# ziyangwang007/CV-SSL-MIS

Hardware: AMD Instinct MI355X
Metric: training images-or-volumes/sec/node (Mean-Teacher step) (higher is better)
Workload: dtype f32

## Files before the change

cv-ssl-mis_amd/csrc/norm_act.hip:

```cpp
#include "common.h"
#include <type_traits>

namespace {

struct Geo {
    int N, C, per_sample;
    long long S;
    long long x_bs;
    int P;
    int nchunks;
    int G;
    int cg;
};

__host__ __device__ inline int pick_P(long long S) {
    long long p = (S + 16383) / 16384;
    if (p < 1) p = 1;
    if (p > 32) p = 32;
    return (int)p;
}

Geo make_geo(int N, int C, long long S, long long x_bs, int per_sample, int cg = 1) {
    Geo g;
    g.N = N; g.C = C; g.S = S; g.x_bs = x_bs; g.per_sample = per_sample; g.cg = cg;
// ... 3 lines not shown
    return g;
}

struct ResArgs {
    const float* r; long long r_bs;
    float* dr; long long dr_bs; int dr_acc;
    int post;
};

struct DropCfg {
    float p;
    unsigned salt;
    const MisStepState* st;
    const float* mask;
};

__device__ __forceinline__ void drop_scale4(const DropCfg& d, unsigned long long idx, unsigned chan, float s[4]) {
    if (d.mask) {
        const float4 m = *reinterpret_cast<const float4*>(d.mask + idx);
        s[0] = m.x; s[1] = m.y; s[2] = m.z; s[3] = m.w;
        return;
    }
    const unsigned long long seed = d.st->seed, off = d.st->offset;
    const float keep = 1.f / (1.f - d.p);
    uint32_t r[4];
    if (d.salt >> 31) {
        mis_philox4((uint32_t)chan, 0x3D0D3D0Du, d.salt, (uint32_t)off, (uint32_t)seed,
                    (uint32_t)(seed >> 32) ^ (uint32_t)(off >> 32), r);
        const float v = mis_u01(r[0]) >= d.p ? keep : 0.f;
        s[0] = s[1] = s[2] = s[3] = v;
// ... 163 lines not shown
                                                        float* __restrict__ y, long long y_bs, ResArgs ra) {
    const int c = blockIdx.y, n = blockIdx.z;
    const int grp = g.per_sample ? (n * g.C + c) / g.cg : c;
    const float sc = (gamma ? gamma[c] : 1.f) * rstd[grp];
    const float sh = (beta ? beta[c] : 0.f) - mean[grp] * sc;
    const float* __restrict__ xb = x + (long long)n * g.x_bs + (long long)c * g.S;
    float* __restrict__ yb = y + (long long)n * y_bs + (long long)c * g.S;
    const unsigned long long lbase = ((unsigned long long)n * g.C + c) * g.S;
    const long long units = g.S >> 2;
    const bool drop = d.p > 0.f;
#pragma unroll
    for (int i = 0; i < APPLY_U; ++i) {
        const long long u = ((long long)blockIdx.x * APPLY_U + i) * 256 + threadIdx.x;
        if (u >= units) break;
        const float4 q = *reinterpret_cast<const float4*>(xb + u * 4);
        float v[4] = {q.x * sc + sh, q.y * sc + sh, q.z * sc + sh, q.w * sc + sh};
        float4 rq = make_float4(0.f, 0.f, 0.f, 0.f);
        if constexpr (RES) {
            rq = *reinterpret_cast<const float4*>(ra.r + (long long)n * ra.r_bs + (long long)c * g.S + u * 4);
            if (!ra.post) { v[0] += rq.x; v[1] += rq.y; v[2] += rq.z; v[3] += rq.w; }
        }
#pragma unroll
        for (int j = 0; j < 4; ++j) v[j] = v[j] > 0.f ? v[j] : v[j] * slope;
        if constexpr (RES) {
            if (ra.post) { v[0] += rq.x; v[1] += rq.y; v[2] += rq.z; v[3] += rq.w; }
        }
        if (drop) {
            float s[4];
            drop_scale4(d, lbase + u * 4, (unsigned)(n * g.C + c), s);
#pragma unroll
            for (int j = 0; j < 4; ++j) v[j] *= s[j];
        }
        *reinterpret_cast<float4*>(yb + u * 4) = make_float4(v[0], v[1], v[2], v[3]);
    }
}

template <int PZ>
__global__ __launch_bounds__(256) void apply_fwd_pool_kernel(const float* __restrict__ x, Geo g,
                                                             const float* __restrict__ mean,
                                                             const float* __restrict__ rstd,
                                                             const float* __restrict__ gamma,
                                                             const float* __restrict__ beta, float slope, DropCfg d,
                                                             float* __restrict__ y, long long y_bs,
                                                             float* __restrict__ pooled, long long p_bs,
                                                             unsigned char* __restrict__ idx, int H, int W) {
    const int Ho = H >> 1, Wo = W >> 1, Wq = Wo >> 2;
    const int pl = blockIdx.x * 256 + threadIdx.x;
    if (pl >= Ho * Wq) return;
    const int zo = blockIdx.y, nc = blockIdx.z;
    const int n = nc / g.C, c = nc - n * g.C;
    const int yo = pl / Wq, xq = pl - yo * Wq;
    const int grp = g.per_sample ? (n * g.C + c) / g.cg : c;
    const float sc = (gamma ? gamma[c] : 1.f) * rstd[grp];
    const float sh = (beta ? beta[c] : 0.f) - mean[grp] * sc;
    const float* __restrict__ xb = x + (long long)n * g.x_bs + (long long)c * g.S;
    float* __restrict__ yb = y + (long long)n * y_bs + (long long)c * g.S;
    const unsigned long long lbase = ((unsigned long long)n * g.C + c) * g.S;
    const bool drop = d.p > 0.f;
    float best[4] = {-INFINITY, -INFINITY, -INFINITY, -INFINITY};
    unsigned bi[4] = {0, 0, 0, 0};
#pragma unroll
    for (int dz = 0; dz < PZ; ++dz)
#pragma unroll
        for (int dy = 0; dy < 2; ++dy) {
            const unsigned e = (unsigned)(((zo * PZ + dz) * H + (yo * 2 + dy)) * W + xq * 8);
            float v[8];
#pragma unroll
            for (int h = 0; h < 2; ++h) {
                const float4 q = *reinterpret_cast<const float4*>(xb + e + 4 * h);
                float t[4] = {q.x * sc + sh, q.y * sc + sh, q.z * sc + sh, q.w * sc + sh};
#pragma unroll
                for (int j = 0; j < 4; ++j) t[j] = t[j] > 0.f ? t[j] : t[j] * slope;
                if (drop) {
                    float s4[4];
                    drop_scale4(d, lbase + e + 4 * h, (unsigned)(n * g.C + c), s4);
#pragma unroll
                    for (int j = 0; j < 4; ++j) t[j] *= s4[j];
                }
                *reinterpret_cast<float4*>(yb + e + 4 * h) = make_float4(t[0], t[1], t[2], t[3]);
#pragma unroll
                for (int j = 0; j < 4; ++j) v[4 * h + j] = t[j];
            }
#pragma unroll
            for (int j = 0; j < 4; ++j)
#pragma unroll
                for (int dx = 0; dx < 2; ++dx) {
                    const float t = v[2 * j + dx];
                    if (t > best[j] || t != t) { best[j] = t; bi[j] = dz * 4 + dy * 2 + dx; }
                }
        }
    const long long So = (long long)gridDim.y * Ho * Wo;
    const unsigned o = (unsigned)((zo * Ho + yo) * Wo + xq * 4);
    *reinterpret_cast<float4*>(pooled + (long long)n * p_bs + (long long)c * So + o) =
        make_float4(best[0], best[1], best[2], best[3]);
    *reinterpret_cast<unsigned*>(idx + (long long)nc * So + o) = bi[0] | (bi[1] << 8) | (bi[2] << 16) | (bi[3] << 24);
}

template <bool DACC, bool RES = false>
__global__ __launch_bounds__(256) void bwd_partial_kernel(const float* __restrict__ x, Geo g,
                                                          const float* __restrict__ da, long long da_bs,
                                                          const float* __restrict__ mean,
                                                          const float* __restrict__ rstd,
                                                          const float* __restrict__ gamma,
                                                          const float* __restrict__ beta, float slope, DropCfg d,
                                                          float2* __restrict__ part, PoolGrad pg, ResArgs ra) {
    __shared__ double red[8];
    const int p = blockIdx.x, k = blockIdx.y, grp = blockIdx.z;
    const int n = g.per_sample ? grp / g.C : k;
    const int c = g.per_sample ? grp % g.C : grp;
    const int sg = g.per_sample ? grp / g.cg : grp;
// ... 414 lines not shown
                                hipStream_t stream) {
    return mis_norm_act_fwd_g(x, x_bs, y, y_bs, N, C, S, per_sample, 1, mean, rstd, gamma, beta, slope, drop_p,
                              drop_salt, state, drop_mask, stream);
}

extern "C" int mis_norm_act_fwd_pool(const float* x, long long x_bs, float* y, long long y_bs, float* pooled,
                                     long long p_bs, unsigned char* idx, int N, int C, int D, int H, int W,
                                     int per_sample, int cg, const float* mean, const float* rstd, const float* gamma,
                                     const float* beta, float slope, float drop_p, unsigned drop_salt,
                                     const MisStepState* state, const float* drop_mask, hipStream_t stream) {
    if (D <= 0 || H <= 0 || W <= 0) return MIS_ERR_ARG;
    const long long S = (long long)D * H * W;
    int st = check_geo(x, N, C, S, x_bs);
    if (st) return st;
    if (cg < 1 || C % cg != 0 || (cg > 1 && !per_sample)) return MIS_ERR_ARG;
    if (!y || !pooled || !idx || !mean || !rstd || y_bs < (long long)C * S) return MIS_ERR_ARG;
    if (W % 8 || H % 2 || (D > 1 && D % 2) || S >= (1LL << 31)) return MIS_ERR_UNSUPPORTED;
    const int pz = D > 1 ? 2 : 1, Do = D / pz;
    const long long So = (long long)Do * (H / 2) * (W / 2);
    if (p_bs < (long long)C * So) return MIS_ERR_ARG;
    if (y_bs % 4 || p_bs % 4 || !aligned16(y) || !aligned16(pooled) || ((uintptr_t)idx & 3)) return MIS_ERR_UNSUPPORTED;
    if (drop_p < 0.f || drop_p >= 1.f || (drop_p > 0.f && !state && !drop_mask)) return MIS_ERR_ARG;
    if (Do > 65535 || (long long)N * C > 65535) return MIS_ERR_UNSUPPORTED;
    const Geo g = make_geo(N, C, S, x_bs, per_sample, cg);
    const DropCfg d{drop_p, drop_salt, state, drop_mask};
    const dim3 grid((unsigned)(((H / 2) * (W / 8) + 255) / 256), Do, N * C);
    if (pz == 2)
        hipLaunchKernelGGL(apply_fwd_pool_kernel<2>, grid, dim3(256), 0, stream, x, g, mean, rstd, gamma, beta, slope, d, y,
                           y_bs, pooled, p_bs, idx, H, W);
    else
        hipLaunchKernelGGL(apply_fwd_pool_kernel<1>, grid, dim3(256), 0, stream, x, g, mean, rstd, gamma, beta, slope, d, y,
                           y_bs, pooled, p_bs, idx, H, W);
    return mis_launch_status();
}

namespace {
int norm_act_bwd_impl(const float* x, long long x_bs, const float* da, long long da_bs, float* dx, long long dx_bs,
                      int N, int C, long long S, int per_sample, int cg, int no_norm, const float* mean,
                      const float* rstd, const float* gamma, const float* beta, float slope, float drop_p,
                      unsigned drop_salt, const MisStepState* state, const float* drop_mask, float* dgamma,
                      float* dbeta, int accumulate_affine, void* workspace, long long workspace_bytes,
                      const PoolGrad& pg, hipStream_t stream, const ResArgs& ra = ResArgs{}) {
    if (S % 4 != 0) {
        if (ra.r) return MIS_ERR_UNSUPPORTED;
        int st = check_geo_small(x, N, C, S, x_bs);
        if (st) return st;
        if (!da || !dx || !mean || !rstd || da_bs < (long long)C * S || dx_bs < (long long)C * S) return MIS_ERR_ARG;
// ... 171 lines not shown

struct HeadArgs {
    const float* x; long long x_bs;
    int N, K, per_sample;
    long long S;
    const float* mean; const float* rstd; const float* gamma; const float* beta;
    float slope;
    const float* w; const float* b;
    float* logits; long long l_bs;
    const float* dl; long long dl_bs;
    float* dx; long long dx_bs;
    float2* part;
    const float2* sums;
    float* hpart;
    int P;
};

template <int C, bool MASK>
__device__ __forceinline__ unsigned long long head_drop_bits(const DropCfg& d, int n, long long S, long long u) {
    unsigned long long bits = ~0ull;
    if (!MASK && d.p > 0.f) {
        bits = 0;
#pragma unroll 1
        for (int c = 0; c < C; ++c) {
            float s[4];
            drop_scale4(d, ((unsigned long long)n * C + c) * S + u * 4, (unsigned)(n * C + c), s);
#pragma unroll
            for (int j = 0; j < 4; ++j) bits |= (unsigned long long)(s[j] != 0.f) << (4 * c + j);
        }
    }
// ... 24 lines not shown
template <int C, int K, bool MASK>
__global__ __launch_bounds__(256) void head_fwd_fused_kernel(const HeadArgs a, DropCfg d) {
    __shared__ float sc[C], sh[C], sw[K * C];
    const int n = blockIdx.y;
    head_coeffs<C>(a, n, sc, sh);
    for (int i = threadIdx.x; i < K * C; i += 256) sw[i] = a.w[i];
    __syncthreads();
    const long long units = a.S >> 2, u = (long long)blockIdx.x * 256 + threadIdx.x;
    if (u >= units) return;
    const float* __restrict__ xb = a.x + (long long)n * a.x_bs + u * 4;
    float4 q[C];
#pragma unroll
    for (int c = 0; c < C; ++c) q[c] = *reinterpret_cast<const float4*>(xb + (long long)c * a.S);
    const float keep = d.p > 0.f ? 1.f / (1.f - d.p) : 1.f;
    const unsigned long long bits = head_drop_bits<C, MASK>(d, n, a.S, u);
    float acc[K][4];
#pragma unroll
    for (int k = 0; k < K; ++k) {
        const float bk = a.b ? a.b[k] : 0.f;
#pragma unroll
        for (int j = 0; j < 4; ++j) acc[k][j] = bk;
    }
#pragma unroll
    for (int c = 0; c < C; ++c) {
        float v[4] = {q[c].x * sc[c] + sh[c], q[c].y * sc[c] + sh[c], q[c].z * sc[c] + sh[c], q[c].w * sc[c] + sh[c]};
#pragma unroll
        for (int j = 0; j < 4; ++j) v[j] = v[j] > 0.f ? v[j] : v[j] * a.slope;
        {
            float s[4];
            head_drop_scale<C, MASK>(d, bits, keep, n, a.S, u, c, s);
// ... 22 lines not shown
    const long long per = (units + a.P - 1) / a.P;
    const long long u0 = p * per, u1 = (u0 + per < units) ? u0 + per : units;
    const float keep = d.p > 0.f ? 1.f / (1.f - d.p) : 1.f;
    constexpr int NV = 2 * C + K * C + K;
    float v[NV];
#pragma unroll
    for (int i = 0; i < NV; ++i) v[i] = 0.f;
    for (long long u = u0 + threadIdx.x; u < u1; u += 256) {
        float4 g4[K];
#pragma unroll
        for (int k = 0; k < K; ++k) {
            g4[k] = *reinterpret_cast<const float4*>(a.dl + (long long)n * a.dl_bs + (long long)k * a.S + u * 4);
            v[2 * C + K * C + k] += (g4[k].x + g4[k].y) + (g4[k].z + g4[k].w);
        }
        const float* __restrict__ xb = a.x + (long long)n * a.x_bs + u * 4;
        const unsigned long long bits = head_drop_bits<C, MASK>(d, n, a.S, u);
#pragma unroll
        for (int c = 0; c < C; ++c) {
            const float4 q = *reinterpret_cast<const float4*>(xb + (long long)c * a.S);
            const float xs[4] = {q.x, q.y, q.z, q.w};
            float s[4];
            head_drop_scale<C, MASK>(d, bits, keep, n, a.S, u, c, s);
            const int grp = a.per_sample ? n * C + c : c;
            const float m = a.mean[grp], rs = a.rstd[grp];
#pragma unroll
            for (int j = 0; j < 4; ++j) {
                const float xh = (xs[j] - m) * rs;
                const float z0 = xs[j] * sc[c] + sh[c];
                const float act = (z0 > 0.f ? z0 : z0 * a.slope) * s[j];
                float dzd = 0.f;
#pragma unroll
// ... 49 lines not shown
__global__ __launch_bounds__(256) void head_bwd_apply_kernel(const HeadArgs a, DropCfg d) {
    __shared__ float sc[C], sh[C], sw[K * C];
    const int n = blockIdx.y;
    head_coeffs<C>(a, n, sc, sh);
    for (int i = threadIdx.x; i < K * C; i += 256) sw[i] = a.w[i];
    __syncthreads();
    const long long units = a.S >> 2, u = (long long)blockIdx.x * 256 + threadIdx.x;
    if (u >= units) return;
    float4 g4[K];
#pragma unroll
    for (int k = 0; k < K; ++k)
        g4[k] = *reinterpret_cast<const float4*>(a.dl + (long long)n * a.dl_bs + (long long)k * a.S + u * 4);
    const float* __restrict__ xb = a.x + (long long)n * a.x_bs + u * 4;
    float* __restrict__ ob = a.dx + (long long)n * a.dx_bs + u * 4;
    const float keep = d.p > 0.f ? 1.f / (1.f - d.p) : 1.f;
    const unsigned long long bits = head_drop_bits<C, MASK>(d, n, a.S, u);
#pragma unroll
    for (int c = 0; c < C; ++c) {
        const float4 q = *reinterpret_cast<const float4*>(xb + (long long)c * a.S);
        const float xs[4] = {q.x, q.y, q.z, q.w};
        float s[4];
        head_drop_scale<C, MASK>(d, bits, keep, n, a.S, u, c, s);
        const int grp = a.per_sample ? n * C + c : c;
        const float m = a.mean[grp], rs = a.rstd[grp];
        const float2 sm = a.sums[grp];
        float o[4];
#pragma unroll
        for (int j = 0; j < 4; ++j) {
            float dzd = 0.f;
#pragma unroll
            for (int k = 0; k < K; ++k) dzd = fmaf(sw[k * C + c], (&g4[k].x)[j], dzd);
// ... 39 lines not shown

constexpr int HEAD_PMUL = 3;

extern "C" int mis_norm_head_eligible(int C, int K) { return C == 16 && K >= 2 && K <= 4; }

extern "C" long long mis_norm_head_workspace_bytes(int N, int C, long long S, int per_sample, int K) {
    if (N <= 0 || C <= 0 || S <= 0 || K <= 0) return MIS_ERR_ARG;
    const long long nb = mis_norm_workspace_bytes(N, C, S, per_sample);
    return nb * HEAD_PMUL + (long long)N * pick_P(S) * HEAD_PMUL * (K * C + K) * 4;
}

extern "C" int mis_norm_head_fwd(const float* x, long long x_bs, int N, int C, long long S, int per_sample,
                                 const float* mean, const float* rstd, const float* gamma, const float* beta,
                                 float slope, float drop_p, unsigned drop_salt, const MisStepState* state,
                                 const float* drop_mask, const float* w, const float* b, int K, float* logits,
                                 long long l_bs, hipStream_t stream) {
    int st = check_geo(x, N, C, S, x_bs);
    if (st) return st;
    if (!mis_norm_head_eligible(C, K) || (per_sample && (gamma || beta))) return MIS_ERR_UNSUPPORTED;
    if (!mean || !rstd || !w || !logits || l_bs < (long long)K * S) return MIS_ERR_ARG;
    if (l_bs % 4 != 0 || !aligned16(logits)) return MIS_ERR_UNSUPPORTED;
    if (drop_p < 0.f || drop_p >= 1.f || (drop_p > 0.f && !state && !drop_mask)) return MIS_ERR_ARG;
    HeadArgs a{};
    a.x = x; a.x_bs = x_bs; a.N = N; a.K = K; a.per_sample = per_sample; a.S = S;
    a.mean = mean; a.rstd = rstd; a.gamma = gamma; a.beta = beta; a.slope = slope; a.w = w; a.b = b;
    a.logits = logits; a.l_bs = l_bs;
    const DropCfg d{drop_p, drop_salt, state, drop_mask};
    return head_launch_fwd<16>(a, d, stream);
}

extern "C" int mis_norm_head_bwd(const float* x, long long x_bs, const float* dlogits, long long dl_bs, float* dx,
                                 long long dx_bs, int N, int C, long long S, int per_sample, const float* mean,
                                 const float* rstd, const float* gamma, const float* beta, float slope, float drop_p,
                                 unsigned drop_salt, const MisStepState* state, const float* drop_mask, const float* w,
                                 int K, float* dgamma, float* dbeta, int accumulate_affine, float* dw, float* db,
                                 int accumulate_w, void* workspace, long long workspace_bytes, hipStream_t stream) {
    int st = check_geo(x, N, C, S, x_bs);
    if (st) return st;
    if (!mis_norm_head_eligible(C, K) || (per_sample && (gamma || beta))) return MIS_ERR_UNSUPPORTED;
    if (!dlogits || !dx || !mean || !rstd || !w || !dw || !workspace) return MIS_ERR_ARG;
    if (dl_bs % 4 != 0 || dx_bs % 4 != 0 || !aligned16(dlogits) || !aligned16(dx)) return MIS_ERR_UNSUPPORTED;
    if (dl_bs < (long long)K * S || dx_bs < (long long)C * S) return MIS_ERR_ARG;
    if (drop_p < 0.f || drop_p >= 1.f || (drop_p > 0.f && !state && !drop_mask)) return MIS_ERR_ARG;
    if (workspace_bytes < mis_norm_head_workspace_bytes(N, C, S, per_sample, K)) return MIS_ERR_WORKSPACE;
    Geo g = make_geo(N, C, S, x_bs, per_sample);
    g.P *= HEAD_PMUL;
    float2* part = reinterpret_cast<float2*>(workspace);
    float2* sums = part + (long long)g.G * g.nchunks * g.P;
    HeadArgs a{};
    a.x = x; a.x_bs = x_bs; a.N = N; a.K = K; a.per_sample = per_sample; a.S = S;
    a.mean = mean; a.rstd = rstd; a.gamma = gamma; a.beta = beta; a.slope = slope; a.w = w;
    a.dl = dlogits; a.dl_bs = dl_bs; a.dx = dx; a.dx_bs = dx_bs;
    a.part = part; a.sums = sums; a.hpart = reinterpret_cast<float*>(sums + g.G); a.P = g.P;
    const DropCfg d{drop_p, drop_salt, state, drop_mask};
    head_launch_partial<16>(a, d, stream);
    hipLaunchKernelGGL(bwd_final_kernel, dim3((g.G + 3) / 4), dim3(256), 0, stream, part, g, sums,
                       per_sample ? nullptr : dgamma, per_sample ? nullptr : dbeta, accumulate_affine);
    hipLaunchKernelGGL(head_final_kernel, dim3(K * C + K), dim3(64), 0, stream, a.hpart, N * g.P, K * C, K, dw, db,
                       accumulate_w);
    head_launch_apply<16>(a, d, stream);
    return mis_launch_status();
}
```

cv-ssl-mis_amd/mis_hip/ops.py:

```python
import ctypes as _ctypes
import os as _os

import torch

from . import lib as _l

_scratch = {}


def _geom(t):
    if t.dim() != 5 or t.dtype != torch.float32:
        raise RuntimeError(f"expected 5-D fp32 [N,C,D,H,W], got {tuple(t.shape)} {t.dtype}")
    if not t.is_cuda:
        _l.require_gpu(t)
    N, C, D, H, W = t.shape
    S = D * H * W
    st = t.stride()
    if C > 1 and st[1] != S or (D > 1 and st[2] != H * W) or (H > 1 and st[3] != W) or (W > 1 and st[4] != 1):
        raise RuntimeError(f"activation view must be dense in (C,D,H,W); strides {st} shape {tuple(t.shape)}")
    bs = st[0] if N > 1 else max(st[0], C * S)
    if bs < C * S:
        bs = C * S
    return N, C, D, H, W, S, bs

# ... 460 lines not shown


def conv_wgrad_cin1_norm(x, da, y, per_sample, mean, rstd, gamma, beta, sums, slope, dw, accumulate=False):
    N, Cin, D, H, W, S, xbs = _geom(x)
    _, Cout, _, _, _, _, ybs = _geom(y)
    ws = _ws("wgrad", "mis_conv_wgrad_workspace_bytes", N, Cin, Cout, D, H, W, 1 if D == 1 else 3, 3, 3)
    _l.launch("mis_conv_wgrad_cin1_norm", x, xbs, _view(da), y, ybs, N, D, H, W, int(per_sample), mean, rstd, gamma, beta, sums,
              slope, dw, ws, int(accumulate))


def norm_head_eligible(C, K, per_sample, gamma, beta, cg=1, no_norm=False):
    return bool(_l.query("mis_norm_head_eligible", C, K)) and cg == 1 and not no_norm and not (
        per_sample and (gamma is not None or beta is not None))


def norm_head_fwd(x, logits, per_sample, mean, rstd, gamma, beta, slope, w, b, drop_p=0.0, drop_salt=0, state=None,
                  drop_mask=None):
    N, C, D, H, W, S, xbs = _geom(x)
    _, K, _, _, _, _, lbs = _geom(logits)
    _l.launch("mis_norm_head_fwd", x, xbs, N, C, S, int(per_sample), mean, rstd, gamma, beta, slope, drop_p, drop_salt, state,
              drop_mask, w, b, K, logits, lbs)


def norm_head_bwd(x, dlogits, dx, per_sample, mean, rstd, gamma, beta, slope, w, dw, db, drop_p=0.0, drop_salt=0,
                  state=None, drop_mask=None, dgamma=None, dbeta=None, accumulate_affine=False, accumulate_w=False):
    N, C, D, H, W, S, xbs = _geom(x)
    _, K, _, _, _, _, dlbs = _geom(dlogits)
    ws = _ws("norm", "mis_norm_head_workspace_bytes", N, C, S, int(per_sample), K)
    _l.launch("mis_norm_head_bwd", x, xbs, dlogits, dlbs, _view(dx), N, C, S, int(per_sample), mean, rstd, gamma, beta, slope,
              drop_p, drop_salt, state, drop_mask, w, K, dgamma, dbeta, int(accumulate_affine), dw, db, int(accumulate_w), ws)


def group_norm_stats(x, cg, eps, mean, rstd):
    N, C, D, H, W, S, xbs = _geom(x)
    G = C // cg
    ws = _ws("norm", "mis_norm_workspace_bytes", N, G, cg * S, 1)
    _l.launch("mis_norm_stats", x, xbs, N, G, cg * S, 1, eps, mean, rstd, None, None, None, 0.0, ws)


def maxpool2_fwd(x, y, idx):
    N, C, D, H, W, S, xbs = _geom(x)
    _l.launch("mis_maxpool2_fwd", x, xbs, _view(y), idx, N, C, D, H, W)


def maxpool2_bwd(dy, idx, dx, accumulate=False):
# ... 541 lines not shown
```

cv-ssl-mis_amd/mis_hip/plan.py:

```python
import itertools
import math
import os

import torch
import torch.nn as nn

from . import lib as _lib
from . import ops, tops
from .dist import param_progress

_net_ids = itertools.count(1)

FUSE_CONV_STATS = os.environ.get("MIS_FUSE_STATS", "1") != "0"
FUSE_HEAD = os.environ.get("MIS_FUSE_HEAD", "1") != "0"
FUSE_FIRST = os.environ.get("MIS_FUSE_FIRST", "1") != "0"
FUSE_POOL = os.environ.get("MIS_FUSE_POOL", "1") != "0"
FUSE_POOL_FWD = os.environ.get("MIS_FUSE_POOL_FWD", "1") != "0"
WGRAD_STREAM = os.environ.get("MIS_WGRAD_STREAM", "1") != "0"
FUSE_DGRAD_NORM = os.environ.get("MIS_FUSE_DGRAD_NORM", "1") != "0"
PROGRESS_SYNC_MAIN = os.environ.get("MIS_PROGRESS_SYNC_MAIN", "0") == "1"
NORM_RES = os.environ.get("MIS_NORM_RES", "1") != "0"


class Buf:

    def __init__(self, parent=None, c0=0):
        self.parent, self.c0 = parent, c0
        self._written = False
        self.g = None

    def grad(self):
        if self.g is None:
# ... 193 lines not shown
        self.drop3d = False
        N, C = x.shape[0], x.shape[1]
        G = N * C // cg if per_sample else C
        self.mean = torch.zeros(G, dtype=torch.float32, device="cuda")
        self.rstd = torch.ones(G, dtype=torch.float32, device="cuda")
        self._p = 0.0
        self._mask = self._state = None
        self.pool = None
        self.sums = None
        self.ext_part = None
        self.ext_tiles, self.ext_ready, self.ext_sums = 0, False, None
        self.res = None
        self.res_post = False
        self.head = None
        self.head_w = self.head_b = None
        self.frozen = False

    def _affine(self):
        return (None if self.gamma is None else self.gamma.data, None if self.beta is None else self.beta.data)

    def _affine_grad(self):
        if self.frozen:
            return (None, None)
        return (None if self.gamma is None else self.gamma.grad, None if self.beta is None else self.beta.grad)

    def fwd(self, ctx):
        if self.no_norm:
            pass
        elif not self.per_sample and not ctx.training:
            ops.norm_stats_from_running(self.running[0], self.running[1], self.eps, self.mean, self.rstd)
# ... 8 lines not shown
                ops.group_norm_stats(self.x.t, self.cg, self.eps, self.mean, self.rstd)
            else:
                ops.norm_stats(self.x.t, self.per_sample, self.eps, self.mean, self.rstd, rm, rv, nbt, self.momentum)
        self._p = self.drop_p if (ctx.training and ctx.dropout) else 0.0
        self._mask = ctx.drop_masks.get(self.site) if (ctx.drop_masks and self._p > 0) else None
        self.salt = ((ctx.rng_stream & 0x7FFF) << 16) | self.site | (0x80000000 if self.drop3d else 0)
        self._state = ctx.state
        if self._p > 0 and self._mask is None and ctx.state is None:
            raise RuntimeError("dropout is active but no device step state was supplied (Ctx.state)")
        if self.res is not None:
            ops.norm_res_act_fwd(self.x.t, self.res.t, self.y.t, self.per_sample, self.mean, self.rstd, *self._affine(),
                                 self.slope, post=self.res_post)
            return
        if self.pool is not None and self.pool.fwd_fused:
            pl = self.pool
            ops.norm_act_fwd_pool(self.x.t, self.y.t, pl.y.t, pl.idx, self.per_sample, self.mean, self.rstd, *self._affine(),
                                  self.slope, self._p, self.salt, self._state, self._mask, cg=self.cg)
            return
        if self.head is not None:
            h = self.head
            ops.norm_head_fwd(self.x.t, h.y.t, self.per_sample, self.mean, self.rstd, *self._affine(), self.slope,
                              h.w.data.view(h.cout, h.cin), None if h.b is None else h.b.data, self._p, self.salt,
                              self._state, self._mask)
            return
        ops.norm_act_fwd(self.x.t, self.y.t, self.per_sample, self.mean, self.rstd, *self._affine(), self.slope, self._p,
                         self.salt, self._state, self._mask, cg=self.cg)

    def bwd(self, ctx):
        assert not self.x.written
        if self.res is not None:
            r = self.res
            ops.norm_res_act_bwd(self.x.t, r.t, self.y.grad(), self.x.grad(), r.grad(), r.written, self.per_sample,
                                 self.mean, self.rstd, *self._affine(), self.slope, *self._affine_grad(), post=self.res_post)
            r.mark_written()
            self.x.mark_written()
            return
        if self.ext_ready:
            self.ext_ready = False
# ... 7 lines not shown
            ops.norm_act_bwd_sums(self.x.t, self.y.grad(), self.per_sample, self.mean, self.rstd, *self._affine(), self.slope,
                                  self.sums, *self._affine_grad())
            return
        if self.pool is not None:
            pl = self.pool
            ops.norm_act_bwd_pool(self.x.t, self.y.grad() if self.y.written else None, pl.y.grad(), pl.idx, self.x.grad(),
                                  self.per_sample, self.mean, self.rstd, *self._affine(), self.slope, self._p, self.salt,
                                  self._state, self._mask, *self._affine_grad(), cg=self.cg)
            self.x.mark_written()
            return
        if self.head is not None:
            h = self.head
            ops.norm_head_bwd(self.x.t, h.y.grad(), self.x.grad(), self.per_sample, self.mean, self.rstd, *self._affine(),
                              self.slope, h.w.data.view(h.cout, h.cin), h.w.grad.view(h.cout, h.cin),
                              h.b.grad if (h.b is not None and h.bias_grad) else None, self._p, self.salt, self._state,
                              self._mask, *self._affine_grad())
            self.x.mark_written()
            return
        ops.norm_act_bwd(self.x.t, self.y.grad(), self.x.grad(), self.per_sample, self.mean, self.rstd, *self._affine(),
                         self.slope, self._p, self.salt, self._state, self._mask, *self._affine_grad(), cg=self.cg,
                         no_norm=self.no_norm)
        self.x.mark_written()


class MaxPoolOp:
    def __init__(self, x, y):
        self.x, self.y = x, y
        self.idx = torch.empty(y.t.numel(), dtype=torch.uint8, device="cuda")
        self.fused_into = None
        self.fwd_fused = False

# ... 447 lines not shown
                self.acts.remove(out)
            return a
        if out is None:
            out = self.new(a.shape[1], a.shape[2:], N=a.shape[0])
        self.ops.append(AddOp(a, b, out))
        return out

    def maxpool(self, x, y):
        op = MaxPoolOp(x, y)
        if FUSE_POOL:
            prod = next((o for o in reversed(self.ops) if type(o) is NormActOp and o.y is x), None)
            N, C, D, H, W = x.shape
            if (prod is not None and prod.pool is None and prod.head is None and prod.sums is None and not prod.no_norm
                    and W % 4 == 0 and H % 2 == 0 and (D == 1 or D % 2 == 0) and D * H * W < 2 ** 31):
                prod.pool, op.fused_into = op, prod
                op.fwd_fused = FUSE_POOL_FWD and D == 1 and W % 8 == 0 and prod is self.ops[-1] and y.parent is None
        self.ops.append(op)
        return y

    def upsample(self, x, y, align_corners, scale=2):
        self.ops.append(UpsampleOp(x, y, align_corners, scale))
        return y

    def gate_map(self, theta, phi, att, psi, phi_b):
        self.ops.append(GateMapOp(theta, phi, att, psi, phi_b))
        return att

    def gate_apply(self, x, att, y):
        self.ops.append(GateApplyOp(x, att, y))
        return y

# ... 425 lines not shown
```

include/mis_hip.h:

```cpp
#ifndef MIS_HIP_H
#define MIS_HIP_H

#include <stdint.h>

#ifdef __cplusplus
extern "C" {
#endif

#define MIS_OK 0
#define MIS_ERR_ARG (-1)
#define MIS_ERR_UNSUPPORTED (-2)
#define MIS_ERR_LAUNCH (-3)
#define MIS_ERR_WORKSPACE (-4)

#ifdef MIS_HIP_BUILD
typedef hipStream_t mis_stream_t;
#else
typedef void* mis_stream_t;
#endif

typedef struct MisStepState {
    uint64_t seed;
    uint64_t offset;
    int64_t iter_num;
// ... 109 lines not shown
                         const float* gamma, const float* beta, float slope, float* dgamma, float* dbeta,
                         int accumulate_affine, int add_after_act, void* workspace, long long workspace_bytes,
                         mis_stream_t stream);
int mis_conv_wgrad_cin1_norm_eligible(int N, int Cout, int D, int H, int W);
int mis_conv_wgrad_cin1_norm(const float* x, long long x_bs, const float* da, long long da_bs, const float* y,
                             long long y_bs, int N, int D, int H, int W, int per_sample, const float* mean,
                             const float* rstd, const float* gamma, const float* beta, const float* sums, float slope,
                             float* dw, float* workspace, long long workspace_bytes, int accumulate,
                             mis_stream_t stream);

int mis_norm_head_eligible(int C, int K);
long long mis_norm_head_workspace_bytes(int N, int C, long long S, int per_sample, int K);
int mis_norm_head_fwd(const float* x, long long x_bs, int N, int C, long long S, int per_sample, const float* mean,
                      const float* rstd, const float* gamma, const float* beta, float slope, float drop_p,
                      unsigned drop_salt, const MisStepState* state, const float* drop_mask, const float* w,
                      const float* b, int K, float* logits, long long l_bs, mis_stream_t stream);
int mis_norm_head_bwd(const float* x, long long x_bs, const float* dlogits, long long dl_bs, float* dx, long long dx_bs,
                      int N, int C, long long S, int per_sample, const float* mean, const float* rstd,
                      const float* gamma, const float* beta, float slope, float drop_p, unsigned drop_salt,
                      const MisStepState* state, const float* drop_mask, const float* w, int K, float* dgamma,
                      float* dbeta, int accumulate_affine, float* dw, float* db, int accumulate_w, void* workspace,
                      long long workspace_bytes, mis_stream_t stream);

int mis_norm_act_fwd_pool(const float* x, long long x_bs, float* y, long long y_bs, float* pooled, long long p_bs,
                          unsigned char* idx, int N, int C, int D, int H, int W, int per_sample, int cg,
                          const float* mean, const float* rstd, const float* gamma, const float* beta, float slope,
                          float drop_p, unsigned drop_salt, const MisStepState* state, const float* drop_mask,
                          mis_stream_t stream);
int mis_norm_act_bwd_pool(const float* x, long long x_bs, const float* da, long long da_bs, const float* dpool,
                          long long dp_bs, const unsigned char* idx, float* dx, long long dx_bs, int N, int C, int D,
                          int H, int W, int per_sample, int cg, const float* mean, const float* rstd,
                          const float* gamma, const float* beta, float slope, float drop_p, unsigned drop_salt,
                          const MisStepState* state, const float* drop_mask, float* dgamma, float* dbeta,
                          int accumulate_affine, void* workspace, long long workspace_bytes, mis_stream_t stream);

int mis_maxpool2_fwd(const float* x, long long x_bs, float* y, long long y_bs, unsigned char* idx, int N, int C,
                     int D, int H, int W, mis_stream_t stream);
// ... 310 lines not shown
```

Baseline: 472.8.

## Fuse 3D norm-act with maxpool forward and cache head dropout bits

Adds a dedicated 3D fused norm+activation+maxpool forward kernel. Each thread handles two output depth slices with float4 loads at W%4 granularity. Fusion is now enabled for volumetric inputs. The pool index write is skipped when no backward pass is needed. The head kernel also stores its Philox-derived dropout bitmask during forward so the two backward kernels read it instead of regenerating it, at the cost of an extra int64 buffer per unit. A residual-free fast path in the apply kernel is split out as well.

Result: faster. 478.0 (median of 6 runs) (+1.1%).

```diff
diff --git a/cv-ssl-mis_amd/csrc/norm_act.hip b/cv-ssl-mis_amd/csrc/norm_act.hip
--- a/cv-ssl-mis_amd/csrc/norm_act.hip
+++ b/cv-ssl-mis_amd/csrc/norm_act.hip
@@ -41,6 +41,11 @@
     const MisStepState* st;
     const float* mask;
 };
+
+__device__ __forceinline__ float mis_norm_act1(float x, float sc, float sh, float slope) {
+    const float v = x * sc + sh;
+    return v > 0.f ? v : v * slope;
+}
 
 __device__ __forceinline__ void drop_scale4(const DropCfg& d, unsigned long long idx, unsigned chan, float s[4]) {
     if (d.mask) {
@@ -234,16 +239,17 @@
         const long long u = ((long long)blockIdx.x * APPLY_U + i) * 256 + threadIdx.x;
         if (u >= units) break;
         const float4 q = *reinterpret_cast<const float4*>(xb + u * 4);
-        float v[4] = {q.x * sc + sh, q.y * sc + sh, q.z * sc + sh, q.w * sc + sh};
-        float4 rq = make_float4(0.f, 0.f, 0.f, 0.f);
+        float v[4];
         if constexpr (RES) {
-            rq = *reinterpret_cast<const float4*>(ra.r + (long long)n * ra.r_bs + (long long)c * g.S + u * 4);
+            v[0] = q.x * sc + sh; v[1] = q.y * sc + sh; v[2] = q.z * sc + sh; v[3] = q.w * sc + sh;
+            const float4 rq = *reinterpret_cast<const float4*>(ra.r + (long long)n * ra.r_bs + (long long)c * g.S + u * 4);
             if (!ra.post) { v[0] += rq.x; v[1] += rq.y; v[2] += rq.z; v[3] += rq.w; }
-        }
-#pragma unroll
-        for (int j = 0; j < 4; ++j) v[j] = v[j] > 0.f ? v[j] : v[j] * slope;
-        if constexpr (RES) {
+#pragma unroll
+            for (int j = 0; j < 4; ++j) v[j] = v[j] > 0.f ? v[j] : v[j] * slope;
             if (ra.post) { v[0] += rq.x; v[1] += rq.y; v[2] += rq.z; v[3] += rq.w; }
+        } else {
+            v[0] = mis_norm_act1(q.x, sc, sh, slope); v[1] = mis_norm_act1(q.y, sc, sh, slope);
+            v[2] = mis_norm_act1(q.z, sc, sh, slope); v[3] = mis_norm_act1(q.w, sc, sh, slope);
         }
         if (drop) {
             float s[4];
@@ -255,7 +261,6 @@
     }
 }
 
-template <int PZ>
 __global__ __launch_bounds__(256) void apply_fwd_pool_kernel(const float* __restrict__ x, Geo g,
                                                              const float* __restrict__ mean,
                                                              const float* __restrict__ rstd,
@@ -280,40 +285,110 @@
     float best[4] = {-INFINITY, -INFINITY, -INFINITY, -INFINITY};
     unsigned bi[4] = {0, 0, 0, 0};
 #pragma unroll
-    for (int dz = 0; dz < PZ; ++dz)
-#pragma unroll
-        for (int dy = 0; dy < 2; ++dy) {
-            const unsigned e = (unsigned)(((zo * PZ + dz) * H + (yo * 2 + dy)) * W + xq * 8);
-            float v[8];
-#pragma unroll
-            for (int h = 0; h < 2; ++h) {
-                const float4 q = *reinterpret_cast<const float4*>(xb + e + 4 * h);
-                float t[4] = {q.x * sc + sh, q.y * sc + sh, q.z * sc + sh, q.w * sc + sh};
-#pragma unroll
-                for (int j = 0; j < 4; ++j) t[j] = t[j] > 0.f ? t[j] : t[j] * slope;
-                if (drop) {
-                    float s4[4];
-                    drop_scale4(d, lbase + e + 4 * h, (unsigned)(n * g.C + c), s4);
-#pragma unroll
-                    for (int j = 0; j < 4; ++j) t[j] *= s4[j];
-                }
-                *reinterpret_cast<float4*>(yb + e + 4 * h) = make_float4(t[0], t[1], t[2], t[3]);
-#pragma unroll
-                for (int j = 0; j < 4; ++j) v[4 * h + j] = t[j];
+    for (int dy = 0; dy < 2; ++dy) {
+        const unsigned e = (unsigned)((zo * H + (yo * 2 + dy)) * W + xq * 8);
+        float v[8];
+#pragma unroll
+        for (int h = 0; h < 2; ++h) {
+            const float4 q = *reinterpret_cast<const float4*>(xb + e + 4 * h);
+            float t[4] = {q.x * sc + sh, q.y * sc + sh, q.z * sc + sh, q.w * sc + sh};
+#pragma unroll
+            for (int j = 0; j < 4; ++j) t[j] = t[j] > 0.f ? t[j] : t[j] * slope;
+            if (drop) {
+                float s4[4];
+                drop_scale4(d, lbase + e + 4 * h, (unsigned)(n * g.C + c), s4);
+#pragma unroll
+                for (int j = 0; j < 4; ++j) t[j] *= s4[j];
             }
-#pragma unroll
-            for (int j = 0; j < 4; ++j)
-#pragma unroll
-                for (int dx = 0; dx < 2; ++dx) {
-                    const float t = v[2 * j + dx];
-                    if (t > best[j] || t != t) { best[j] = t; bi[j] = dz * 4 + dy * 2 + dx; }
-                }
-        }
+            *reinterpret_cast<float4*>(yb + e + 4 * h) = make_float4(t[0], t[1], t[2], t[3]);
+#pragma unroll
+            for (int j = 0; j < 4; ++j) v[4 * h + j] = t[j];
+        }
+#pragma unroll
+        for (int j = 0; j < 4; ++j)
+#pragma unroll
+            for (int dx = 0; dx < 2; ++dx) {
+                const float t = v[2 * j + dx];
+                if (t > best[j] || t != t) { best[j] = t; bi[j] = dy * 2 + dx; }
+            }
+    }
     const long long So = (long long)gridDim.y * Ho * Wo;
     const unsigned o = (unsigned)((zo * Ho + yo) * Wo + xq * 4);
     *reinterpret_cast<float4*>(pooled + (long long)n * p_bs + (long long)c * So + o) =
         make_float4(best[0], best[1], best[2], best[3]);
-    *reinterpret_cast<unsigned*>(idx + (long long)nc * So + o) = bi[0] | (bi[1] << 8) | (bi[2] << 16) | (bi[3] << 24);
+    if (idx)
+        *reinterpret_cast<unsigned*>(idx + (long long)nc * So + o) = bi[0] | (bi[1] << 8) | (bi[2] << 16) | (bi[3] << 24);
+}
+
+constexpr int POOL3_ZB = 2;
+
+__global__ __launch_bounds__(256) void apply_fwd_pool3d_kernel(const float* __restrict__ x, Geo g,
+                                                               const float* __restrict__ mean,
+                                                               const float* __restrict__ rstd,
+                                                               const float* __restrict__ gamma,
+                                                               const float* __restrict__ beta, float slope, DropCfg d,
+                                                               float* __restrict__ y, long long y_bs,
+                                                               float* __restrict__ pooled, long long p_bs,
+                                                               unsigned char* __restrict__ idx, int D, int H, int W) {
+    constexpr int ZB = POOL3_ZB;
+    const unsigned Do = (unsigned)D >> 1, Ho = (unsigned)H >> 1, Wo = (unsigned)W >> 1, Wq = (unsigned)W >> 2;
+    const unsigned Zg = (Do + ZB - 1) / ZB;
+    const unsigned t = blockIdx.x * 256u + threadIdx.x;
+    if (t >= Zg * Ho * Wq) return;
+    const unsigned r = t / Wq, xq = t - r * Wq;
+    const unsigned zg = r / Ho, yo = r - zg * Ho;
+    const int nc = blockIdx.y;
+    const int n = nc / g.C, c = nc - n * g.C;
+    const int grp = g.per_sample ? (n * g.C + c) / g.cg : c;
+    const float sc = (gamma ? gamma[c] : 1.f) * rstd[grp];
+    const float sh = (beta ? beta[c] : 0.f) - mean[grp] * sc;
+    const float* __restrict__ xb = x + (long long)n * g.x_bs + (long long)c * g.S;
+    float* __restrict__ yb = y + (long long)n * y_bs + (long long)c * g.S;
+    const unsigned long long lbase = ((unsigned long long)n * g.C + c) * g.S;
+    const bool drop = d.p > 0.f;
+    const unsigned So = Do * Ho * Wo;
+    float4 q[ZB][4];
+#pragma unroll
+    for (int i = 0; i < ZB; ++i) {
+        const unsigned zo = zg * ZB + i;
+#pragma unroll
+        for (int k = 0; k < 4; ++k) {
+            q[i][k] = make_float4(0.f, 0.f, 0.f, 0.f);
+            if (zo < Do)
+                q[i][k] = *reinterpret_cast<const float4*>(xb + ((2 * zo + (k >> 1)) * (unsigned)H + 2 * yo + (k & 1)) * (unsigned)W +
+                                                           4 * xq);
+        }
+    }
+#pragma unroll
+    for (int i = 0; i < ZB; ++i) {
+        const unsigned zo = zg * ZB + i;
+        if (zo >= Do) break;
+        float best[2] = {-INFINITY, -INFINITY};
+        unsigned bi[2] = {0, 0};
+#pragma unroll
+        for (int k = 0; k < 4; ++k) {
+            const unsigned e = ((2 * zo + (k >> 1)) * (unsigned)H + 2 * yo + (k & 1)) * (unsigned)W + 4 * xq;
+            float v[4] = {mis_norm_act1(q[i][k].x, sc, sh, slope), mis_norm_act1(q[i][k].y, sc, sh, slope),
+                          mis_norm_act1(q[i][k].z, sc, sh, slope), mis_norm_act1(q[i][k].w, sc, sh, slope)};
+            if (drop) {
+                float s4[4];
+                drop_scale4(d, lbase + e, (unsigned)(n * g.C + c), s4);
+#pragma unroll
+                for (int j = 0; j < 4; ++j) v[j] *= s4[j];
+            }
+            *reinterpret_cast<float4*>(yb + e) = make_float4(v[0], v[1], v[2], v[3]);
+#pragma unroll
+            for (int j = 0; j < 2; ++j)
+#pragma unroll
+                for (int dx = 0; dx < 2; ++dx) {
+                    const float tv = v[2 * j + dx];
+                    if (tv > best[j] || tv != tv) { best[j] = tv; bi[j] = k * 2 + dx; }
+                }
+        }
+        const unsigned o = (zo * Ho + yo) * Wo + 2 * xq;
+        *reinterpret_cast<float2*>(pooled + (long long)n * p_bs + (long long)c * So + o) = make_float2(best[0], best[1]);
+        if (idx) *reinterpret_cast<unsigned short*>(idx + (long long)nc * So + o) = (unsigned short)(bi[0] | (bi[1] << 8));
+    }
 }
 
 template <bool DACC, bool RES = false>
@@ -758,8 +833,8 @@
     int st = check_geo(x, N, C, S, x_bs);
     if (st) return st;
     if (cg < 1 || C % cg != 0 || (cg > 1 && !per_sample)) return MIS_ERR_ARG;
-    if (!y || !pooled || !idx || !mean || !rstd || y_bs < (long long)C * S) return MIS_ERR_ARG;
-    if (W % 8 || H % 2 || (D > 1 && D % 2) || S >= (1LL << 31)) return MIS_ERR_UNSUPPORTED;
+    if (!y || !pooled || !mean || !rstd || y_bs < (long long)C * S) return MIS_ERR_ARG;
+    if (W % (D > 1 ? 4 : 8) || H % 2 || (D > 1 && D % 2) || S >= (1LL << 31)) return MIS_ERR_UNSUPPORTED;
     const int pz = D > 1 ? 2 : 1, Do = D / pz;
     const long long So = (long long)Do * (H / 2) * (W / 2);
     if (p_bs < (long long)C * So) return MIS_ERR_ARG;
@@ -768,13 +843,15 @@
     if (Do > 65535 || (long long)N * C > 65535) return MIS_ERR_UNSUPPORTED;
     const Geo g = make_geo(N, C, S, x_bs, per_sample, cg);
     const DropCfg d{drop_p, drop_salt, state, drop_mask};
-    const dim3 grid((unsigned)(((H / 2) * (W / 8) + 255) / 256), Do, N * C);
-    if (pz == 2)
-        hipLaunchKernelGGL(apply_fwd_pool_kernel<2>, grid, dim3(256), 0, stream, x, g, mean, rstd, gamma, beta, slope, d, y,
+    if (pz == 2) {
+        const long long threads = mis_cdiv(Do, POOL3_ZB) * (H / 2) * (W / 4);
+        hipLaunchKernelGGL(apply_fwd_pool3d_kernel, dim3((unsigned)mis_cdiv(threads, 256), N * C), dim3(256), 0, stream, x, g,
+                           mean, rstd, gamma, beta, slope, d, y, y_bs, pooled, p_bs, idx, D, H, W);
+    } else {
+        const dim3 grid((unsigned)(((H / 2) * (W / 8) + 255) / 256), 1, N * C);
+        hipLaunchKernelGGL(apply_fwd_pool_kernel, grid, dim3(256), 0, stream, x, g, mean, rstd, gamma, beta, slope, d, y,
                            y_bs, pooled, p_bs, idx, H, W);
-    else
-        hipLaunchKernelGGL(apply_fwd_pool_kernel<1>, grid, dim3(256), 0, stream, x, g, mean, rstd, gamma, beta, slope, d, y,
-                           y_bs, pooled, p_bs, idx, H, W);
+    }
     return mis_launch_status();
 }
 
@@ -976,6 +1053,7 @@
     const float2* sums;
     float* hpart;
     int P;
+    unsigned long long* bits;
 };
 
 template <int C, bool MASK>
@@ -1030,6 +1108,7 @@
     for (int c = 0; c < C; ++c) q[c] = *reinterpret_cast<const float4*>(xb + (long long)c * a.S);
     const float keep = d.p > 0.f ? 1.f / (1.f - d.p) : 1.f;
     const unsigned long long bits = head_drop_bits<C, MASK>(d, n, a.S, u);
+    if (!MASK && a.bits) a.bits[(long long)n * units + u] = bits;
     float acc[K][4];
 #pragma unroll
     for (int k = 0; k < K; ++k) {
@@ -1082,7 +1161,8 @@
             v[2 * C + K * C + k] += (g4[k].x + g4[k].y) + (g4[k].z + g4[k].w);
         }
         const float* __restrict__ xb = a.x + (long long)n * a.x_bs + u * 4;
-        const unsigned long long bits = head_drop_bits<C, MASK>(d, n, a.S, u);
+        const unsigned long long bits =
+            (!MASK && a.bits) ? a.bits[(long long)n * units + u] : head_drop_bits<C, MASK>(d, n, a.S, u);
 #pragma unroll
         for (int c = 0; c < C; ++c) {
             const float4 q = *reinterpret_cast<const float4*>(xb + (long long)c * a.S);
@@ -1162,7 +1242,8 @@
     const float* __restrict__ xb = a.x + (long long)n * a.x_bs + u * 4;
     float* __restrict__ ob = a.dx + (long long)n * a.dx_bs + u * 4;
     const float keep = d.p > 0.f ? 1.f / (1.f - d.p) : 1.f;
-    const unsigned long long bits = head_drop_bits<C, MASK>(d, n, a.S, u);
+    const unsigned long long bits =
+        (!MASK && a.bits) ? a.bits[(long long)n * units + u] : head_drop_bits<C, MASK>(d, n, a.S, u);
 #pragma unroll
     for (int c = 0; c < C; ++c) {
         const float4 q = *reinterpret_cast<const float4*>(xb + (long long)c * a.S);
@@ -1232,17 +1313,17 @@
                                  const float* mean, const float* rstd, const float* gamma, const float* beta,
                                  float slope, float drop_p, unsigned drop_salt, const MisStepState* state,
                                  const float* drop_mask, const float* w, const float* b, int K, float* logits,
-                                 long long l_bs, hipStream_t stream) {
+                                 long long l_bs, unsigned long long* drop_bits, hipStream_t stream) {
     int st = check_geo(x, N, C, S, x_bs);
     if (st) return st;
     if (!mis_norm_head_eligible(C, K) || (per_sample && (gamma || beta))) return MIS_ERR_UNSUPPORTED;
     if (!mean || !rstd || !w || !logits || l_bs < (long long)K * S) return MIS_ERR_ARG;
-    if (l_bs % 4 != 0 || !aligned16(logits)) return MIS_ERR_UNSUPPORTED;
+    if (l_bs % 4 != 0 || !aligned16(logits) || ((uintptr_t)drop_bits & 7)) return MIS_ERR_UNSUPPORTED;
     if (drop_p < 0.f || drop_p >= 1.f || (drop_p > 0.f && !state && !drop_mask)) return MIS_ERR_ARG;
     HeadArgs a{};
     a.x = x; a.x_bs = x_bs; a.N = N; a.K = K; a.per_sample = per_sample; a.S = S;
     a.mean = mean; a.rstd = rstd; a.gamma = gamma; a.beta = beta; a.slope = slope; a.w = w; a.b = b;
-    a.logits = logits; a.l_bs = l_bs;
+    a.logits = logits; a.l_bs = l_bs; a.bits = drop_bits;
     const DropCfg d{drop_p, drop_salt, state, drop_mask};
     return head_launch_fwd<16>(a, d, stream);
 }
@@ -1252,12 +1333,14 @@
                                  const float* rstd, const float* gamma, const float* beta, float slope, float drop_p,
                                  unsigned drop_salt, const MisStepState* state, const float* drop_mask, const float* w,
                                  int K, float* dgamma, float* dbeta, int accumulate_affine, float* dw, float* db,
-                                 int accumulate_w, void* workspace, long long workspace_bytes, hipStream_t stream) {
+                                 int accumulate_w, const unsigned long long* drop_bits, void* workspace,
+                                 long long workspace_bytes, hipStream_t stream) {
     int st = check_geo(x, N, C, S, x_bs);
     if (st) return st;
     if (!mis_norm_head_eligible(C, K) || (per_sample && (gamma || beta))) return MIS_ERR_UNSUPPORTED;
     if (!dlogits || !dx || !mean || !rstd || !w || !dw || !workspace) return MIS_ERR_ARG;
-    if (dl_bs % 4 != 0 || dx_bs % 4 != 0 || !aligned16(dlogits) || !aligned16(dx)) return MIS_ERR_UNSUPPORTED;
+    if (dl_bs % 4 != 0 || dx_bs % 4 != 0 || !aligned16(dlogits) || !aligned16(dx) || ((uintptr_t)drop_bits & 7))
+        return MIS_ERR_UNSUPPORTED;
     if (dl_bs < (long long)K * S || dx_bs < (long long)C * S) return MIS_ERR_ARG;
     if (drop_p < 0.f || drop_p >= 1.f || (drop_p > 0.f && !state && !drop_mask)) return MIS_ERR_ARG;
     if (workspace_bytes < mis_norm_head_workspace_bytes(N, C, S, per_sample, K)) return MIS_ERR_WORKSPACE;
@@ -1270,6 +1353,7 @@
     a.mean = mean; a.rstd = rstd; a.gamma = gamma; a.beta = beta; a.slope = slope; a.w = w;
     a.dl = dlogits; a.dl_bs = dl_bs; a.dx = dx; a.dx_bs = dx_bs;
     a.part = part; a.sums = sums; a.hpart = reinterpret_cast<float*>(sums + g.G); a.P = g.P;
+    a.bits = const_cast<unsigned long long*>(drop_bits);
     const DropCfg d{drop_p, drop_salt, state, drop_mask};
     head_launch_partial<16>(a, d, stream);
     hipLaunchKernelGGL(bwd_final_kernel, dim3((g.G + 3) / 4), dim3(256), 0, stream, part, g, sums,
diff --git a/cv-ssl-mis_amd/mis_hip/ops.py b/cv-ssl-mis_amd/mis_hip/ops.py
--- a/cv-ssl-mis_amd/mis_hip/ops.py
+++ b/cv-ssl-mis_amd/mis_hip/ops.py
@@ -498,21 +498,29 @@
         per_sample and (gamma is not None or beta is not None))
 
 
+def norm_head_bits(x):
+    N, C, D, H, W, S, _ = _geom(x)
+    return torch.empty(N * (S // 4), dtype=torch.int64, device=x.device)
+
+
 def norm_head_fwd(x, logits, per_sample, mean, rstd, gamma, beta, slope, w, b, drop_p=0.0, drop_salt=0, state=None,
-                  drop_mask=None):
+                  drop_mask=None, bits=None):
     N, C, D, H, W, S, xbs = _geom(x)
     _, K, _, _, _, _, lbs = _geom(logits)
+    assert bits is None or (bits.dtype == torch.int64 and bits.is_contiguous() and bits.numel() >= N * (S // 4))
     _l.launch("mis_norm_head_fwd", x, xbs, N, C, S, int(per_sample), mean, rstd, gamma, beta, slope, drop_p, drop_salt, state,
-              drop_mask, w, b, K, logits, lbs)
+              drop_mask, w, b, K, logits, lbs, bits)
 
 
 def norm_head_bwd(x, dlogits, dx, per_sample, mean, rstd, gamma, beta, slope, w, dw, db, drop_p=0.0, drop_salt=0,
-                  state=None, drop_mask=None, dgamma=None, dbeta=None, accumulate_affine=False, accumulate_w=False):
+                  state=None, drop_mask=None, dgamma=None, dbeta=None, accumulate_affine=False, accumulate_w=False, bits=None):
     N, C, D, H, W, S, xbs = _geom(x)
     _, K, _, _, _, _, dlbs = _geom(dlogits)
     ws = _ws("norm", "mis_norm_head_workspace_bytes", N, C, S, int(per_sample), K)
+    assert bits is None or (bits.dtype == torch.int64 and bits.is_contiguous() and bits.numel() >= N * (S // 4))
     _l.launch("mis_norm_head_bwd", x, xbs, dlogits, dlbs, _view(dx), N, C, S, int(per_sample), mean, rstd, gamma, beta, slope,
-              drop_p, drop_salt, state, drop_mask, w, K, dgamma, dbeta, int(accumulate_affine), dw, db, int(accumulate_w), ws)
+              drop_p, drop_salt, state, drop_mask, w, K, dgamma, dbeta, int(accumulate_affine), dw, db, int(accumulate_w), bits,
+              ws)
 
 
 def group_norm_stats(x, cg, eps, mean, rstd):
diff --git a/cv-ssl-mis_amd/mis_hip/plan.py b/cv-ssl-mis_amd/mis_hip/plan.py
--- a/cv-ssl-mis_amd/mis_hip/plan.py
+++ b/cv-ssl-mis_amd/mis_hip/plan.py
@@ -16,6 +16,8 @@
 FUSE_FIRST = os.environ.get("MIS_FUSE_FIRST", "1") != "0"
 FUSE_POOL = os.environ.get("MIS_FUSE_POOL", "1") != "0"
 FUSE_POOL_FWD = os.environ.get("MIS_FUSE_POOL_FWD", "1") != "0"
+FUSE_POOL_FWD_3D = os.environ.get("MIS_FUSE_POOL_FWD_3D", "1") != "0"
+HEAD_DROP_BITS = os.environ.get("MIS_HEAD_DROP_BITS", "1") != "0"
 WGRAD_STREAM = os.environ.get("MIS_WGRAD_STREAM", "1") != "0"
 FUSE_DGRAD_NORM = os.environ.get("MIS_FUSE_DGRAD_NORM", "1") != "0"
 PROGRESS_SYNC_MAIN = os.environ.get("MIS_PROGRESS_SYNC_MAIN", "0") == "1"
@@ -239,6 +241,8 @@
         self.res_post = False
         self.head = None
         self.head_w = self.head_b = None
+        self.head_bits = None
+        self._bits = None
         self.frozen = False
 
     def _affine(self):
@@ -277,14 +281,20 @@
             return
         if self.pool is not None and self.pool.fwd_fused:
             pl = self.pool
-            ops.norm_act_fwd_pool(self.x.t, self.y.t, pl.y.t, pl.idx, self.per_sample, self.mean, self.rstd, *self._affine(),
-                                  self.slope, self._p, self.salt, self._state, self._mask, cg=self.cg)
+            ops.norm_act_fwd_pool(self.x.t, self.y.t, pl.y.t, None if (ctx.no_backward and pl.y.shape[2] > 1) else pl.idx,
+                                  self.per_sample, self.mean, self.rstd, *self._affine(), self.slope, self._p, self.salt,
+                                  self._state, self._mask, cg=self.cg)
             return
         if self.head is not None:
             h = self.head
+            self._bits = None
+            if HEAD_DROP_BITS and self._p > 0 and self._mask is None and not ctx.no_backward:
+                if self.head_bits is None:
+                    self.head_bits = ops.norm_head_bits(self.x.t)
+                self._bits = self.head_bits
             ops.norm_head_fwd(self.x.t, h.y.t, self.per_sample, self.mean, self.rstd, *self._affine(), self.slope,
                               h.w.data.view(h.cout, h.cin), None if h.b is None else h.b.data, self._p, self.salt,
-                              self._state, self._mask)
+                              self._state, self._mask, bits=self._bits)
             return
         ops.norm_act_fwd(self.x.t, self.y.t, self.per_sample, self.mean, self.rstd, *self._affine(), self.slope, self._p,
                          self.salt, self._state, self._mask, cg=self.cg)
@@ -322,7 +332,7 @@
             ops.norm_head_bwd(self.x.t, h.y.grad(), self.x.grad(), self.per_sample, self.mean, self.rstd, *self._affine(),
                               self.slope, h.w.data.view(h.cout, h.cin), h.w.grad.view(h.cout, h.cin),
                               h.b.grad if (h.b is not None and h.bias_grad) else None, self._p, self.salt, self._state,
-                              self._mask, *self._affine_grad())
+                              self._mask, *self._affine_grad(), bits=self._bits)
             self.x.mark_written()
             return
         ops.norm_act_bwd(self.x.t, self.y.grad(), self.x.grad(), self.per_sample, self.mean, self.rstd, *self._affine(),
@@ -800,7 +810,8 @@
             if (prod is not None and prod.pool is None and prod.head is None and prod.sums is None and not prod.no_norm
                     and W % 4 == 0 and H % 2 == 0 and (D == 1 or D % 2 == 0) and D * H * W < 2 ** 31):
                 prod.pool, op.fused_into = op, prod
-                op.fwd_fused = FUSE_POOL_FWD and D == 1 and W % 8 == 0 and prod is self.ops[-1] and y.parent is None
+                fusable = (W % 8 == 0) if D == 1 else (FUSE_POOL_FWD_3D and D % 2 == 0)
+                op.fwd_fused = FUSE_POOL_FWD and fusable and prod is self.ops[-1] and y.parent is None
         self.ops.append(op)
         return y
 
diff --git a/include/mis_hip.h b/include/mis_hip.h
--- a/include/mis_hip.h
+++ b/include/mis_hip.h
@@ -147,13 +147,15 @@
 int mis_norm_head_fwd(const float* x, long long x_bs, int N, int C, long long S, int per_sample, const float* mean,
                       const float* rstd, const float* gamma, const float* beta, float slope, float drop_p,
                       unsigned drop_salt, const MisStepState* state, const float* drop_mask, const float* w,
-                      const float* b, int K, float* logits, long long l_bs, mis_stream_t stream);
+                      const float* b, int K, float* logits, long long l_bs, unsigned long long* drop_bits,
+                      mis_stream_t stream);
 int mis_norm_head_bwd(const float* x, long long x_bs, const float* dlogits, long long dl_bs, float* dx, long long dx_bs,
                       int N, int C, long long S, int per_sample, const float* mean, const float* rstd,
                       const float* gamma, const float* beta, float slope, float drop_p, unsigned drop_salt,
                       const MisStepState* state, const float* drop_mask, const float* w, int K, float* dgamma,
-                      float* dbeta, int accumulate_affine, float* dw, float* db, int accumulate_w, void* workspace,
-                      long long workspace_bytes, mis_stream_t stream);
+                      float* dbeta, int accumulate_affine, float* dw, float* db, int accumulate_w,
+                      const unsigned long long* drop_bits, void* workspace, long long workspace_bytes,
+                      mis_stream_t stream);
 
 int mis_norm_act_fwd_pool(const float* x, long long x_bs, float* y, long long y_bs, float* pooled, long long p_bs,
                           unsigned char* idx, int N, int C, int D, int H, int W, int per_sample, int cg,
```
